# mlpc-ucsd/BDM

Measured on AMD Instinct MI355X. Metric: sampled shapes/sec (4096 pts, 1000 DDPM steps), higher is better.
Workload: dtype f32

## Files before the change

bdm_amd/csrc/sparse_conv_os.hip:

```cpp
#include <stdlib.h>

#include "../../include/bdm_hip.h"
#include "common.h"

using namespace bdm;

#include "sparse_h2_common.h"

#define OS_PAIRS 14

typedef __attribute__((ext_vector_type(4))) float f32x4a;
typedef float f32x4v_t __attribute__((ext_vector_type(4)));


#define TILE_REC 16
#define DILH_XCAP 1376

static void sconv_dil_geometry(int r, int half_tile, int *tile, int *xcap, int *tiles_max) {
  if (half_tile > 0) {
    *tile = half_tile;
    *xcap = DILH_XCAP;
  } else {
    *tile = r == 32 ? 512 : (r == 16 ? 256 : 128);
    *xcap = 3 * r * r;
  }
  *tiles_max = (r * r * r) / *tile + r;
}

__global__ __launch_bounds__(1024) void vox_dilate_kernel(int r, int n_dil_max, int tile, int xcap, int tiles_max, int half_form,
                                                          const int *__restrict__ cnt, int thr, int *__restrict__ dil_list,
                                                          int *__restrict__ dil_index, int *__restrict__ plane_start,
                                                          int *__restrict__ tile_start, int *__restrict__ class_count) {
  extern __shared__ unsigned bits[];
  const int bi = blockIdx.x, tid = threadIdx.x, T = blockDim.x, lane = tid & 63, wave = tid >> 6;
  const int r2 = r * r, r3 = r2 * r;
  unsigned *occ = bits;
  int *wtot = reinterpret_cast<int *>(bits + r2);
  int *ps_o = wtot + 32, *ps_d = ps_o + (r + 2);
  const int *c = cnt + (size_t)bi * r3;
  for (int v0 = wave * 64; v0 < r3; v0 += 8 * T) {
    int cv[8];
#pragma unroll
    for (int u = 0; u < 8; ++u) cv[u] = v0 + u * T < r3 ? c[v0 + u * T + lane] : thr;
#pragma unroll
    for (int u = 0; u < 8; ++u) {
      const int vu = v0 + u * T;
      if (vu < r3) {
        const unsigned long long m = __ballot(cv[u] > thr);
        const int rows = 64 / r;
        if (lane < rows) occ[vu / r + lane] = (unsigned)((m >> (lane * r)) & (r == 32 ? 0xffffffffull : ((1ull << r) - 1ull)));
      }
    }
  }
  __syncthreads();
  const unsigned full = r == 32 ? 0xffffffffu : ((1u << r) - 1u);
  unsigned d = 0u;
  int nocc_row = 0;
  if (tid < r2) {
    const int x = tid / r, y = tid % r;
    for (int dx = -1; dx <= 1; ++dx)
      for (int dy = -1; dy <= 1; ++dy) {
        const int gx = x + dx, gy = y + dy;
        if (gx < 0 || gx >= r || gy < 0 || gy >= r) continue;
        const unsigned m = occ[gx * r + gy];
        d |= m | (m << 1) | (m >> 1);
      }
    d &= full;
    nocc_row = __popc(occ[tid]);
  }
  int incl_d = __popc(d), incl_o = nocc_row;
  const int mine_d = incl_d, mine_o = incl_o;
#pragma unroll
  for (int o = 1; o < 64; o <<= 1) {
    const int td = __shfl_up(incl_d, o, 64), to = __shfl_up(incl_o, o, 64);
    if (lane >= o) { incl_d += td; incl_o += to; }
  }
  if (lane == 63) { wtot[wave] = incl_d; wtot[16 + wave] = incl_o; }
  __syncthreads();
  int off_d = 0, off_o = 0, tot_d = 0, tot_o = 0;
  for (int w = 0; w < (T >> 6); ++w) {
    if (w < wave) { off_d += wtot[w]; off_o += wtot[16 + w]; }
    tot_d += wtot[w]; tot_o += wtot[16 + w];
  }
  unsigned *drow = bits + r2 + 32 + 2 * (r + 2);
  int *drun = reinterpret_cast<int *>(drow + r2);
  int *rs = drun + r2;
  if (tid < r2) {
    const int run = off_d + incl_d - mine_d;
    if (tid % r == 0) { ps_o[tid / r] = off_o + incl_o - mine_o; ps_d[tid / r] = run; }
    drow[tid] = d;
    drun[tid] = run;
    rs[tid] = off_o + incl_o - mine_o;
  }
  if (tid == 0) rs[r2] = tot_o;
  __syncthreads();
  {
    int *dl = dil_list + (size_t)bi * n_dil_max;
    int *di = dil_index + (size_t)bi * r3;
    for (int v = tid; v < r3; v += T) {
      const int row = v / r, z = v - row * r;
      const unsigned m = drow[row];
      const bool in = (m >> z) & 1u;
      const int rank = drun[row] + __popc(m & ((1u << z) - 1u));
      const bool ok = in && rank < n_dil_max;
      di[v] = ok ? rank : -1;
      if (ok) dl[rank] = v;
    }
  }
  if (class_count != nullptr) {
    __shared__ int s_cls[27];
    if (tid < 27) s_cls[tid] = 0;
    __syncthreads();
    if (tid < r2) {
      const int x = tid / r, y = tid % r;
      const int cx = x == 0 ? 0 : (x == r - 1 ? 2 : 1), cy = y == 0 ? 0 : (y == r - 1 ? 2 : 1);
      const unsigned out = ~d & full;
      const int lo = out & 1u, hi = (out >> (r - 1)) & 1u, mid = __popc(out) - lo - hi;
      if (lo) atomicAdd(&s_cls[(cx * 3 + cy) * 3 + 0], lo);
      if (mid) atomicAdd(&s_cls[(cx * 3 + cy) * 3 + 1], mid);
      if (hi) atomicAdd(&s_cls[(cx * 3 + cy) * 3 + 2], hi);
    }
    __syncthreads();
    if (tid < 27) class_count[(size_t)bi * 27 + tid] = s_cls[tid];
  }
  if (tid == 0) { ps_o[r] = ps_o[r + 1] = tot_o; ps_d[r] = ps_d[r + 1] = tot_d; }
  __syncthreads();
  for (int x = tid; x < r + 2; x += T) plane_start[(size_t)bi * (r + 2) + x] = ps_o[x];
  if (half_form) {
    __threadfence();
    __syncthreads();
    const int *dl = dil_list + (size_t)bi * n_dil_max;
    const int nd = min(tot_d, n_dil_max), nt_flat = (nd + tile - 1) / tile;
    int pieces = 0, j = 0, jend = 0, x0 = 0, x1 = 0;
    if (tid < nt_flat) {
      j = tid * tile; jend = min(j + tile, nd);
      x0 = dl[j] / r2; x1 = dl[jend - 1] / r2;
      pieces = (x0 == x1 || rs[min(x1 + 2, r) * r] - rs[max(x0 - 1, 0) * r] <= xcap) ? 1 : x1 - x0 + 1;
    }
    int incl = pieces;
#pragma unroll
    for (int o = 1; o < 64; o <<= 1) {
      const int tq = __shfl_up(incl, o, 64);
      if (lane >= o) incl += tq;
    }
    if (lane == 63) wtot[wave] = incl;
    __syncthreads();
    int off = 0, nt = 0;
    for (int w = 0; w < (T >> 6); ++w) {
      if (w < wave) off += wtot[w];
      nt += wtot[w];
    }
    nt = min(nt, tiles_max);
    off += incl - pieces;
    for (int k = 0; k < pieces; ++k) {
      const int t = off + k;
      if (t >= tiles_max) break;
      int a = j, e_ = jend, xa = x0, xb = x1;
      if (pieces > 1) { xa = xb = x0 + k; a = max(j, ps_d[xa]); e_ = min(jend, ps_d[xa + 1]); if (e_ < a) e_ = a; }
      int lo[3] = {0, 0, 0}, nn[3] = {0, 0, 0};
      if (e_ > a) {
        if (xa == xb) {
          const int y0 = (dl[a] / r) % r, y1 = (dl[e_ - 1] / r) % r;
          for (int dx = 0; dx < 3; ++dx) {
            const int px = xa + dx - 1;
            if (px < 0 || px >= r) continue;
            lo[dx] = rs[px * r + max(y0 - 1, 0)];
            nn[dx] = rs[px * r + min(y1 + 1, r - 1) + 1] - lo[dx];
          }
        } else {
          lo[0] = rs[max(xa - 1, 0) * r];
          nn[0] = rs[min(xb + 2, r) * r] - lo[0];
        }
      }
      int *e = tile_start + ((size_t)bi * tiles_max + t) * TILE_REC;
      const int vf = t == 0 ? 0 : (a < nd ? dl[a] : r3), ve = (t + 1 < nt && e_ < nd) ? dl[e_] : r3;
      e[0] = a; e[1] = e_; e[2] = vf; e[3] = ve; e[4] = lo[0]; e[5] = nn[0]; e[6] = (xa << 8) | xb; e[7] = nt;
      e[8] = lo[1]; e[9] = nn[1]; e[10] = lo[2]; e[11] = nn[2]; e[12] = tile; e[13] = e[14] = e[15] = 0;
    }
    for (int t = nt + tid; t < tiles_max; t += T) {
      int *e = tile_start + ((size_t)bi * tiles_max + t) * TILE_REC;
      const bool first_empty = t == 0;
      e[0] = nd; e[1] = nd; e[2] = first_empty ? 0 : r3; e[3] = r3; e[4] = 0; e[5] = 0; e[6] = 0; e[7] = nt;
      for (int q = 8; q < TILE_REC; ++q) e[q] = q == 12 ? tile : 0;
    }
    return;
  }
  int *tinfo = reinterpret_cast<int *>(occ);
  __shared__ int s_tiles, s_cut;
  if (tid == 0) s_cut = 0;
  __syncthreads();
  {
    const int nd = min(tot_d, n_dil_max), nt_flat = (nd + tile - 1) / tile;
    if (tid < nt_flat && tid < tiles_max) {
      const int j = tid * tile, jend = min(j + tile, nd);
      int lo = 0, hi = r;
      while (hi - lo > 1) { const int mid = (lo + hi) >> 1; if (ps_d[mid] <= j) lo = mid; else hi = mid; }
      const int x0 = lo;
      lo = x0; hi = r;
      while (hi - lo > 1) { const int mid = (lo + hi) >> 1; if (ps_d[mid] <= jend - 1) lo = mid; else hi = mid; }
      const int x1 = lo;
      if (x1 > x0 && ps_o[min(x1 + 2, r)] - ps_o[max(x0 - 1, 0)] > xcap) s_cut = 1;
      tinfo[2 * tid] = j; tinfo[2 * tid + 1] = (x0 << 8) | x1;
    }
    if (tid == 0) { tinfo[2 * min(nt_flat, tiles_max)] = nd; s_tiles = min(nt_flat, tiles_max); }
  }
  __syncthreads();
  if (tid == 0 && s_cut) {
    const int nd = min(tot_d, n_dil_max);
    int t = 0, j = 0, x0 = 0;
    while (j < nd && t < tiles_max) {
      while (ps_d[x0 + 1] <= j) ++x0;
      int jend = min(j + tile, nd), x1 = x0;
      while (ps_d[x1 + 1] < jend) ++x1;
      while (x1 > x0 && ps_o[min(x1 + 2, r)] - ps_o[max(x0 - 1, 0)] > xcap) { jend = ps_d[x1]; --x1; }
      tinfo[2 * t] = j; tinfo[2 * t + 1] = (x0 << 8) | x1;
      ++t;
      j = jend;
    }
    tinfo[2 * t] = nd;
    s_tiles = t;
  }
  __threadfence();
  __syncthreads();
  const int nt = s_tiles, nd = min(tot_d, n_dil_max);
  for (int t = tid; t < tiles_max; t += T) {
    int *e = tile_start + ((size_t)bi * tiles_max + t) * TILE_REC;
    const int *dl = dil_list + (size_t)bi * n_dil_max;
    int j0 = nd, jn = nd, vf = r3, ve = r3, klo = 0, nr = 0;
    if (t < nt) {
      j0 = tinfo[2 * t]; jn = tinfo[2 * t + 2];
      const int x0 = tinfo[2 * t + 1] >> 8, x1 = tinfo[2 * t + 1] & 255;
      vf = t == 0 ? 0 : dl[j0];
      ve = t + 1 < nt ? dl[jn] : r3;
      klo = ps_o[max(x0 - 1, 0)];
      nr = min(ps_o[min(x1 + 2, r)] - klo, xcap);
    } else if (t == 0) { vf = 0; ve = r3; }
    e[0] = j0; e[1] = jn; e[2] = vf; e[3] = ve; e[4] = klo; e[5] = nr; e[6] = t < nt ? tinfo[2 * t + 1] : 0; e[7] = nt;
    for (int q = 8; q < TILE_REC; ++q) e[q] = 0;
  }
}

#ifdef BDM_EXPERIMENTAL
static bool half_tile_ok(int r, int tile) { return tile == 0 || ((r == 16 || r == 32) && (tile == 64 || tile == 128 || tile == 256)) || (r == 8 && (tile == 64 || tile == 128)); }
#else
static bool half_tile_ok(int, int tile) { return tile == 0; }
#endif

extern "C" int bdm_voxel_dilate_slices(int r, int tile) {
  int tl, xcap, tiles_max;
  sconv_dil_geometry(r, half_tile_ok(r, tile) ? tile : 0, &tl, &xcap, &tiles_max);
  return tiles_max;
}

static int voxel_dilate_launch(int b, int r, int n_dil_max, const int *src, int thr, int *dil_list, int *dil_index, int *plane_start,
                               int *tile_start, int *class_count, int half_tile, void *stream) {
  BDM_REQUIRE(b >= 0 && (r == 8 || r == 16 || r == 32) && n_dil_max >= 1 && src && dil_list && dil_index && plane_start && tile_start,
              "voxel_dilate: bad arguments (r in {8, 16, 32})");
  BDM_REQUIRE(half_tile_ok(r, half_tile), "voxel_dilate: tile %d unsupported (0 = full tiles; 64 / 128 / 256: EXPERIMENTAL=1 builds)", half_tile);
  if (b == 0) return BDM_OK;
  int tile, xcap, tiles_max;
  sconv_dil_geometry(r, half_tile, &tile, &xcap, &tiles_max);
  BDM_REQUIRE(cdiv(r * r * r, tile) <= 1024, "voxel_dilate: more flat tiles than threads");
  const size_t smem = sizeof(unsigned) * (4 * (size_t)r * r + 1 + 32 + 2 * (r + 2));
  hipLaunchKernelGGL(vox_dilate_kernel, dim3(b), dim3(1024), smem, (hipStream_t)stream, r, n_dil_max, tile, xcap, tiles_max,
                     half_tile > 0 ? 1 : 0, src, thr, dil_list, dil_index, plane_start, tile_start, class_count);
  return launch_status("voxel_dilate");
}

extern "C" int bdm_voxel_dilate(int b, int r, int n_dil_max, const int *cnt, int *dil_list, int *dil_index, int *plane_start,
                                int *tile_start, int tile, void *stream) {
  return voxel_dilate_launch(b, r, n_dil_max, cnt, 0, dil_list, dil_index, plane_start, tile_start, nullptr, tile, stream);
}

extern "C" int bdm_voxel_dilate_again(int b, int r, int n_dil_max, const int *dil_index_in, int *dil_list, int *dil_index,
                                      int *plane_start, int *tile_start, int *class_count, int tile, void *stream) {
  BDM_REQUIRE(class_count != nullptr, "voxel_dilate_again: class_count is NULL");
  return voxel_dilate_launch(b, r, n_dil_max, dil_index_in, -1, dil_list, dil_index, plane_start, tile_start, class_count, tile, stream);
}

#ifdef DIL_TIMING
__device__ long long *g_dil_ts = nullptr;
extern "C" int bdm_debug_dil_timestamps(long long *buf) { return hipMemcpyToSymbol(HIP_SYMBOL(g_dil_ts), &buf, sizeof(buf)) == hipSuccess ? 0 : 1; }
#define DIL_STAMP(i) do { if (g_dil_ts && tid == 0) { g_dil_ts[(size_t)item * 8 + (i)] = wall_clock64();                                  \
    if ((i) == 0) g_dil_ts[(size_t)item * 8 + 7] = (long long)__builtin_amdgcn_s_getreg(63492) | ((long long)__builtin_amdgcn_s_getreg(63508) << 32); } } while (0)
#else
#define DIL_STAMP(i)
#endif

template <int MT, int NT, int NW, int R, bool H2IN>
__global__ __launch_bounds__(NW * 64) void sconv_dil_kernel(
    int C8, int Cout, int n_max, int n_dil_max, int xcap, const float4 *__restrict__ xr, const float *__restrict__ amax,
    const float4 *__restrict__ xconst, float x_inv_scale,
    const int *__restrict__ occ_index, const int *__restrict__ dil_list, const int *__restrict__ dil_index,
    const int *__restrict__ tile_start, const float4 *__restrict__ wq,
    const float *__restrict__ inv_scale, const float *__restrict__ bias, float *__restrict__ y, int compact, int gn_cg,
    double *__restrict__ gn_partial, int gn_slices, int nb_shapes, int ncb, int tiles_max, int *__restrict__ work_counter) {
  extern __shared__ __align__(16) float4 smem4[];
  constexpr int BM = 16 * MT, TILE = NT * NW * 16;
  constexpr int R2 = R * R, R3 = R2 * R;
  constexpr int NT_ = NW * 64;
  constexpr int WV = OS_PAIRS * 2 * 2 * BM, WI = (WV + NT_ - 1) / NT_;
  constexpr int NQ = OS_PAIRS / 2;
  constexpr int PF = MT * NT >= 16 ? 1 : 2;
  constexpr int NBLK = NT * NW, NB = MT * 4 * 2;
  float4 *Ws = smem4;
  float4 *Xs = smem4 + WV;
  const int XS = xcap + 128;
  __shared__ int s_item;
  __shared__ float s_osc[64], s_obi[64];

  const int tid0 = threadIdx.x;
  const int G = gn_partial != nullptr ? Cout / gn_cg : 0, S = gn_slices;
  const int items = tiles_max * ncb * nb_shapes;
  for (;;) {
    int tid = tid0;
    asm volatile("" : "+v"(tid));
    const int lane = tid & 63, wave = tid >> 6, l16 = lane & 15, kg = lane >> 4;
    __syncthreads();
    if (tid == 0) s_item = atomicAdd(work_counter, 1);
    __syncthreads();
    const int item = s_item;
    if (item >= items) break;
    const int bi = item % nb_shapes, m0 = ((item / nb_shapes) % ncb) * BM, tile = item / (nb_shapes * ncb);
  const int4 *te = reinterpret_cast<const int4 *>(tile_start + ((size_t)bi * tiles_max + tile) * TILE_REC);
  const int4 ta = te[0], tb = te[1];
  const int j0 = ta.x, jn = ta.y, v_first = ta.z, v_end = ta.w, k_lo = tb.x;
  const int tiles_live = tb.w, tile_x0 = tb.z >> 8, tile_x1 = tb.z & 255;
  if (tile >= max(tiles_live, 1)) {
    if (gn_partial != nullptr) {
      const int ngt = BM / gn_cg;
      if (tid < ngt && m0 + tid * gn_cg < Cout) {
        double *dst = gn_partial + (((size_t)bi * G + m0 / gn_cg + tid) * S + tile) * 2;
        dst[0] = 0.0; dst[1] = 0.0;
      }
    }
    continue;
  }
  DIL_STAMP(0);
  const int *dl = dil_list + (size_t)bi * n_dil_max;
  const bool nothing = jn <= j0;
  const int nrows = nothing ? 0 : tb.y;

  const float sx = H2IN ? 1.0f / x_inv_scale : act_scale_from_max(amax[bi]);
  if (tid < BM) {
    const int m = min(m0 + tid, Cout - 1);
    s_osc[tid] = inv_scale[m] * (1.0f / sx);
    s_obi[tid] = bias ? bias[m] : 0.f;
  }
  const float4 *wbase = Ws + ((kg >> 1) * 4 + (kg & 1)) * BM + l16;
  f32x4a acc[MT][NT];
#pragma unroll
  for (int a = 0; a < MT; ++a)
#pragma unroll
    for (int q = 0; q < NT; ++q) acc[a][q] = f32x4a{0.f, 0.f, 0.f, 0.f};
  f32x4v_t cr = {0.f, 0.f, 0.f, 0.f};

  const float4 *xb = xr + (size_t)bi * C8 * n_max * 2;
  typedef f32x4v_t f32x4v;
  f32x4v xa[PF][2], wr[WI];
  auto load_chunk = [&](int c8) {
#pragma unroll
    for (int u = 0; u < PF; ++u) {
      const int row = min(tid + u * NT_, max(nrows - 1, 0));
      if (H2IN) {
        const f32x4v *src = reinterpret_cast<const f32x4v *>(xr + (((size_t)bi * C8 + c8) * 2) * n_max + k_lo + row);
        xa[u][0] = src[0];
        xa[u][1] = src[n_max];
      } else {
        const f32x4v *src = reinterpret_cast<const f32x4v *>(xb + ((size_t)c8 * n_max + k_lo + row) * 2);
        xa[u][0] = src[0];
        xa[u][1] = src[1];
      }
    }
    if (H2IN && tid < 128) cr = *reinterpret_cast<const f32x4v *>(xconst + ((size_t)bi * C8 + c8) * 2 + (tid >> 6));
#pragma unroll
    for (int i = 0; i < WI; ++i) {
      const int e = tid + i * NT_;
      const int m = e % BM, psh = e / BM;
      const bool ok = e < WV && m0 + m < Cout;
      wr[i] = *reinterpret_cast<const f32x4v *>(&wq[ok ? (unsigned)((c8 * (OS_PAIRS * 4) + psh) * Cout + m0 + m) : 0u]);
    }
  };
  auto put = [&](int row, const float4 &p, const float4 &q) {
    if (H2IN) {
      Xs[row] = p;
      Xs[XS + row] = q;
    } else {
      f16x8 hi, lo;
      split_record(p, q, sx, hi, lo);
      *reinterpret_cast<f16x8 *>(&Xs[row]) = hi;
      *reinterpret_cast<f16x8 *>(&Xs[XS + row]) = lo;
    }
  };
  auto store_chunk = [&](int c8) {
#pragma unroll
    for (int u = 0; u < PF; ++u)
      if (tid + u * NT_ < nrows) {
        const float4 p = make_float4(xa[u][0][0], xa[u][0][1], xa[u][0][2], xa[u][0][3]);
        const float4 q = make_float4(xa[u][1][0], xa[u][1][1], xa[u][1][2], xa[u][1][3]);
        put(tid + u * NT_, p, q);
      }
    for (int row0 = tid + PF * NT_; row0 < nrows; row0 += 2 * NT_) {
      const int row1 = row0 + NT_, rc1 = min(row1, nrows - 1);
      float4 a0, a1, b0, b1;
      if (H2IN) {
        const float4 *src = xr + (((size_t)bi * C8 + c8) * 2) * n_max + k_lo;
        a0 = src[row0]; a1 = src[n_max + row0]; b0 = src[rc1]; b1 = src[n_max + rc1];
      } else {
        const float4 *src = xb + ((size_t)c8 * n_max + k_lo) * 2;
        a0 = src[2 * row0]; a1 = src[2 * row0 + 1]; b0 = src[2 * rc1]; b1 = src[2 * rc1 + 1];
      }
      put(row0, a0, a1);
      if (row1 < nrows) put(row1, b0, b1);
    }
    if (H2IN && tid < 128) *reinterpret_cast<f32x4v *>(&Xs[(tid >> 6) * XS + xcap + 64 + (tid & 63)]) = cr;
#pragma unroll
    for (int i = 0; i < WI; ++i) {
      const int e = tid + i * NT_;
      if (e < WV) *reinterpret_cast<f32x4v *>(&Ws[e]) = wr[i];
    }
  };

  if (!nothing) load_chunk(0);

  int rec[NT][NQ];
  unsigned amask = 0u;
  {
    const int pl0 = max(tile_x0 - 1, 0), pl1 = min(tile_x1 + 1, R - 1), n_oi = (pl1 - pl0 + 1) * R2;
    const bool staged = !nothing && n_oi * (int)sizeof(int) <= 2 * XS * (int)sizeof(float4);
    int *s_oi = reinterpret_cast<int *>(Xs);
    const int *oi = occ_index + (size_t)bi * R3;
    int vq[NT];
#pragma unroll
    for (int q = 0; q < NT; ++q) {
      const int j = j0 + (q * NW + wave) * 16 + l16;
      vq[q] = j < jn ? dl[j] : -1;
    }
    if (staged) {
      const int4 *src = reinterpret_cast<const int4 *>(oi + pl0 * R2);
      for (int e = tid; e < n_oi / 4; e += NT_) reinterpret_cast<int4 *>(s_oi)[e] = src[e];
      __syncthreads();
    }
#pragma unroll
    for (int q = 0; q < NT; ++q) {
      const int v = vq[q];
      const int vx = v / R2, vy = (v / R) % R, vz = v % R;
#pragma unroll
      for (int Q = 0; Q < NQ; ++Q) {
        const int t = 4 * Q + kg;
        int k = -1;
        bool inside = false;
        if (v >= 0 && t < 27) {
          const int gx = vx + t / 9 - 1, gy = vy + (t / 3) % 3 - 1, gz = vz + t % 3 - 1;
          inside = gx >= 0 && gx < R && gy >= 0 && gy < R && gz >= 0 && gz < R;
          if (inside) k = staged ? s_oi[((gx - pl0) * R + gy) * R + gz] : oi[(gx * R + gy) * R + gz];
        }
        const bool here = k >= k_lo && k - k_lo < nrows;
        const bool live = here || (H2IN && inside);
        if (__ballot(live) != 0ull) amask |= 1u << (Q * NT + q);
        rec[q][Q] = here ? k - k_lo : ((H2IN && inside) ? xcap + 64 + lane : xcap + lane);
      }
    }
    amask = __builtin_amdgcn_readfirstlane(amask);
  }
  DIL_STAMP(1);
  if (!nothing) {
    for (int c8 = 0; c8 < C8; ++c8) {
      __syncthreads();
      if (c8 == 0) DIL_STAMP(2);
      if (c8 == 0 && tid < 128) Xs[(tid >> 6) * XS + xcap + (tid & 63)] = make_float4(0.f, 0.f, 0.f, 0.f);
      store_chunk(c8);
      __syncthreads();
      if (c8 == 0) DIL_STAMP(3);
      if (c8 == 1) DIL_STAMP(4);
      if (c8 + 1 < C8) load_chunk(c8 + 1);
#pragma unroll
      for (int Q = 0; Q < NQ; ++Q) {
        const unsigned qm = (amask >> (Q * NT)) & ((1u << NT) - 1u);
        if (qm == 0u) continue;
        f16x8 fa[MT][2];
#pragma unroll
        for (int s = 0; s < 2; ++s)
#pragma unroll
          for (int mt = 0; mt < MT; ++mt) {
            const float4 t = wbase[Q * 8 * BM + s * 2 * BM + mt * 16];
            fa[mt][s] = *reinterpret_cast<const f16x8 *>(&t);
          }
#pragma unroll
        for (int q = 0; q < NT; ++q) {
          f16x8 fb[2];
#pragma unroll
          for (int s = 0; s < 2; ++s) {
            const float4 t = Xs[s * XS + rec[q][Q]];
            fb[s] = *reinterpret_cast<const f16x8 *>(&t);
          }
#pragma unroll
          for (int term = 0; term < 3; ++term)
#pragma unroll
            for (int mt = 0; mt < MT; ++mt)
              acc[mt][q] = __builtin_amdgcn_mfma_f32_16x16x32_f16(fa[mt][term == 0 ? 1 : 0], fb[term == 1 ? 1 : 0], acc[mt][q], 0, 0, 0);
        }
      }
    }
  }

  DIL_STAMP(5);
  __syncthreads();
  float *red = reinterpret_cast<float *>(smem4);
  float *otile = red + (NBLK + 1) * NB;
#pragma unroll
  for (int mt = 0; mt < MT; ++mt)
#pragma unroll
    for (int q = 0; q < NT; ++q) {
      const int jl = (q * NW + wave) * 16 + l16;
      const bool live = j0 + jl < jn;
      float bs = 0.f, bq = 0.f;
      f32x4a o = f32x4a{0.f, 0.f, 0.f, 0.f};
#pragma unroll
      for (int i = 0; i < 4; ++i) {
        const int m = m0 + mt * 16 + 4 * kg + i;
        if (m < Cout && live) {
          const float v = acc[mt][q][i] * s_osc[mt * 16 + 4 * kg + i] + s_obi[mt * 16 + 4 * kg + i];
          o[i] = v;
          bs += v;
          bq = __builtin_fmaf(v, v, bq);
        }
      }
      if (live) {
        const int mb = m0 + mt * 16 + 4 * kg;
        if (compact) {
          float *dst = y + ((size_t)bi * n_dil_max + j0 + jl) * Cout + mb;
          if (mb + 3 < Cout && (Cout & 3) == 0) *reinterpret_cast<f32x4a *>(dst) = o;
          else
            for (int i = 0; i < 4 && mb + i < Cout; ++i) dst[i] = o[i];
        } else {
#pragma unroll
          for (int i = 0; i < 4; ++i) otile[(mt * 16 + 4 * kg + i) * TILE + jl] = o[i];
        }
      }
      if (gn_partial != nullptr) {
        bs = row16_sum(bs);
        bq = row16_sum(bq);
        if (l16 == 0) {
          const int nb = q * NW + wave;
          red[nb * NB + (mt * 4 + kg) * 2 + 0] = bs;
          red[nb * NB + (mt * 4 + kg) * 2 + 1] = bq;
        }
      }
    }
  if (gn_partial != nullptr || !compact) __syncthreads();
  if (!compact) {
    const int *di = dil_index + (size_t)bi * R3;
    float *yb = y + (size_t)bi * Cout * R3;
    for (int m = wave; m < BM; m += NW) {
      if (m0 + m >= Cout) break;
      const float bv = bias ? bias[m0 + m] : 0.f;
      float *row = yb + (size_t)(m0 + m) * R3;
      for (int v = v_first + lane; v < v_end; v += 64) {
        const int j = di[v];
        row[v] = j >= 0 ? otile[m * TILE + (j - j0)] : bv;
      }
    }
  }
  if (gn_partial != nullptr) {
    float *red2 = red + NBLK * NB;
    for (int e = tid; e < NB; e += NT_) {
      float a = 0.f;
#pragma unroll
      for (int j = 0; j < NBLK; ++j) a += red[j * NB + e];
      red2[e] = a;
    }
    __syncthreads();
    const int ngt = BM / gn_cg;
    if (tid < ngt && m0 + tid * gn_cg < Cout) {
      double a = 0.0, qq = 0.0;
      const int nb4 = gn_cg / 4;
      for (int j = 0; j < nb4; ++j) {
        a += (double)red2[(tid * nb4 + j) * 2 + 0];
        qq += (double)red2[(tid * nb4 + j) * 2 + 1];
      }
      const double nfill = H2IN ? 0.0 : (double)((v_end - v_first) - (jn - j0));
      for (int c = 0; c < gn_cg; ++c) {
        const double bv = bias ? (double)bias[m0 + tid * gn_cg + c] : 0.0;
        a += nfill * bv;
        qq += nfill * bv * bv;
      }
      double *dst = gn_partial + (((size_t)bi * G + m0 / gn_cg + tid) * S + tile) * 2;
      dst[0] = a;
      dst[1] = qq;
    }
  }
  DIL_STAMP(6);
  }
}


#ifdef BDM_EXPERIMENTAL
template <int MT, int NT, int R, bool H2IN>
__global__ __launch_bounds__(256, 2) void sconv_dilh_kernel(
    int C8, int Cout, int n_max, int n_dil_max, const float4 *__restrict__ xr, const float *__restrict__ amax,
    const float4 *__restrict__ xconst, float x_inv_scale,
    const int *__restrict__ occ_index, const int *__restrict__ dil_list, const int *__restrict__ dil_index,
    const int *__restrict__ tile_start, const float4 *__restrict__ wq,
    const float *__restrict__ inv_scale, const float *__restrict__ bias, float *__restrict__ y, int compact, int gn_cg,
    double *__restrict__ gn_partial, int gn_slices, int nb_shapes, int ncb, int tiles_max, int *__restrict__ work_counter) {
  extern __shared__ __align__(16) float4 smem4[];
  constexpr int NW = 4, NT_ = NW * 64;
  constexpr int BM = 16 * MT, TILE = NT * NW * 16;
  constexpr int R2 = R * R, R3 = R2 * R;
  constexpr int NQ = OS_PAIRS / 2;
  constexpr int PF = 3;
  constexpr int NBLK = NT * NW, NB = MT * 4 * 2;
  constexpr int XCAP = DILH_XCAP, XS = XCAP + 128;
  float4 *Xs = smem4;
  __shared__ int s_item;
  __shared__ float s_osc[64], s_obi[64];

  const int tid0 = threadIdx.x;
  const int G = gn_partial != nullptr ? Cout / gn_cg : 0, S = gn_slices;
  const int items = tiles_max * ncb * nb_shapes;
  for (;;) {
    int tid = tid0;
    asm volatile("" : "+v"(tid));
    const int lane = tid & 63, wave = tid >> 6, l16 = lane & 15, kg = lane >> 4;
    __syncthreads();
    if (tid == 0) s_item = atomicAdd(work_counter, 1);
    __syncthreads();
    const int item = s_item;
    if (item >= items) break;
    const int bi = item % nb_shapes, m0 = ((item / nb_shapes) % ncb) * BM, tile = item / (nb_shapes * ncb);
    const int4 *te = reinterpret_cast<const int4 *>(tile_start + ((size_t)bi * tiles_max + tile) * TILE_REC);
    const int4 ta = te[0], tb = te[1], tc = te[2];
    const int j0 = ta.x, jn = ta.y, v_first = ta.z, v_end = ta.w;
    const int tiles_live = tb.w, tile_x0 = tb.z >> 8, tile_x1 = tb.z & 255;
    if (tile >= max(tiles_live, 1)) {
      if (gn_partial != nullptr) {
        const int ngt = BM / gn_cg;
        if (tid < ngt && m0 + tid * gn_cg < Cout) {
          double *dst = gn_partial + (((size_t)bi * G + m0 / gn_cg + tid) * S + tile) * 2;
          dst[0] = 0.0; dst[1] = 0.0;
        }
      }
      continue;
    }
    DIL_STAMP(0);
    const int *dl = dil_list + (size_t)bi * n_dil_max;
    const bool nothing = jn <= j0;
    const int lo0 = tb.x, n0 = nothing ? 0 : tb.y, lo1 = tc.x, n1 = nothing ? 0 : tc.y, lo2 = tc.z, n2 = nothing ? 0 : tc.w;
    const int n01 = n0 + n1, nrows = min(n01 + n2, XCAP);
    auto grow = [&](int i) { return i < n0 ? lo0 + i : (i < n01 ? lo1 + (i - n0) : lo2 + (i - n01)); };

    const float sx = H2IN ? 1.0f / x_inv_scale : act_scale_from_max(amax[bi]);
    if (tid < BM) {
      const int m = min(m0 + tid, Cout - 1);
      s_osc[tid] = inv_scale[m] * (1.0f / sx);
      s_obi[tid] = bias ? bias[m] : 0.f;
    }
    const __amdgpu_buffer_rsrc_t wrsrc = __builtin_amdgcn_make_buffer_rsrc(const_cast<float4 *>(wq), 0, C8 * (OS_PAIRS * 4) * Cout * 16, 0x00020000);
    const int wlane = (((kg >> 1) * 4 + (kg & 1)) * Cout + m0 + l16) * 16;
    f32x4a acc[MT][NT];
#pragma unroll
    for (int a = 0; a < MT; ++a)
#pragma unroll
      for (int q = 0; q < NT; ++q) acc[a][q] = f32x4a{0.f, 0.f, 0.f, 0.f};
    typedef f32x4v_t f32x4v;
    f32x4v cr = {0.f, 0.f, 0.f, 0.f};
    f32x4v xa[PF][2];
    const float4 *xb = xr + (size_t)bi * C8 * n_max * 2;

    auto load_x = [&](int c8) {
#pragma unroll
      for (int u = 0; u < PF; ++u) {
        const int g = grow(min(tid + u * NT_, max(nrows - 1, 0)));
        if (H2IN) {
          const f32x4v *src = reinterpret_cast<const f32x4v *>(xr + (((size_t)bi * C8 + c8) * 2) * n_max + g);
          xa[u][0] = src[0];
          xa[u][1] = src[n_max];
        } else {
          const f32x4v *src = reinterpret_cast<const f32x4v *>(xb + ((size_t)c8 * n_max + g) * 2);
          xa[u][0] = src[0];
          xa[u][1] = src[1];
        }
      }
      if (H2IN && tid < 128) cr = *reinterpret_cast<const f32x4v *>(xconst + ((size_t)bi * C8 + c8) * 2 + (tid >> 6));
    };
    auto put = [&](int row, const float4 &p, const float4 &q) {
      if (H2IN) {
        Xs[row] = p;
        Xs[XS + row] = q;
      } else {
        f16x8 hi, lo;
        split_record(p, q, sx, hi, lo);
        *reinterpret_cast<f16x8 *>(&Xs[row]) = hi;
        *reinterpret_cast<f16x8 *>(&Xs[XS + row]) = lo;
      }
    };
    auto store_x = [&](int c8) {
      const int rows_w = nrows;
#pragma unroll
      for (int u = 0; u < PF; ++u)
        if (tid + u * NT_ < rows_w) {
          const float4 p = make_float4(xa[u][0][0], xa[u][0][1], xa[u][0][2], xa[u][0][3]);
          const float4 q = make_float4(xa[u][1][0], xa[u][1][1], xa[u][1][2], xa[u][1][3]);
          put(tid + u * NT_, p, q);
        }
      for (int row0 = tid + PF * NT_; row0 < rows_w; row0 += 2 * NT_) {
        const int row1 = row0 + NT_, rc1 = min(row1, rows_w - 1);
        const int g0 = grow(row0), g1 = grow(rc1);
        float4 a0, a1, b0, b1;
        if (H2IN) {
          const float4 *src = xr + (((size_t)bi * C8 + c8) * 2) * n_max;
          a0 = src[g0]; a1 = src[n_max + g0]; b0 = src[g1]; b1 = src[n_max + g1];
        } else {
          const float4 *src = xb + ((size_t)c8 * n_max) * 2;
          a0 = src[2 * g0]; a1 = src[2 * g0 + 1]; b0 = src[2 * g1]; b1 = src[2 * g1 + 1];
        }
        put(row0, a0, a1);
        if (row1 < rows_w) put(row1, b0, b1);
      }
      if (H2IN && tid < 128) *reinterpret_cast<f32x4v *>(&Xs[(tid >> 6) * XS + XCAP + 64 + (tid & 63)]) = cr;
    };

    if (!nothing) load_x(0);

    int rec[NT][NQ];
    unsigned amask = 0u;
    {
      const int pl0 = max(tile_x0 - 1, 0), pl1 = min(tile_x1 + 1, R - 1), n_oi = (pl1 - pl0 + 1) * R2;
      const bool staged = !nothing && n_oi * (int)sizeof(int) <= 2 * XS * (int)sizeof(float4);
      int *s_oi = reinterpret_cast<int *>(Xs);
      const int *oi = occ_index + (size_t)bi * R3;
      int vq[NT];
#pragma unroll
      for (int q = 0; q < NT; ++q) {
        const int j = j0 + (q * NW + wave) * 16 + l16;
        vq[q] = j < jn ? dl[j] : -1;
      }
      if (staged) {
        const int4 *src = reinterpret_cast<const int4 *>(oi + pl0 * R2);
        for (int e = tid; e < n_oi / 4; e += NT_) reinterpret_cast<int4 *>(s_oi)[e] = src[e];
        __syncthreads();
      }
#pragma unroll
      for (int q = 0; q < NT; ++q) {
        const int v = vq[q];
        const int vx = v / R2, vy = (v / R) % R, vz = v % R;
#pragma unroll
        for (int Q = 0; Q < NQ; ++Q) {
          const int t = 4 * Q + kg;
          int k = -1;
          bool inside = false;
          if (v >= 0 && t < 27) {
            const int gx = vx + t / 9 - 1, gy = vy + (t / 3) % 3 - 1, gz = vz + t % 3 - 1;
            inside = gx >= 0 && gx < R && gy >= 0 && gy < R && gz >= 0 && gz < R;
            if (inside) k = staged ? s_oi[((gx - pl0) * R + gy) * R + gz] : oi[(gx * R + gy) * R + gz];
          }
          int row = -1;
          if (k >= 0) {
            if ((unsigned)(k - lo0) < (unsigned)n0) row = k - lo0;
            else if ((unsigned)(k - lo1) < (unsigned)n1) row = n0 + (k - lo1);
            else if ((unsigned)(k - lo2) < (unsigned)n2) row = n01 + (k - lo2);
          }
          const bool here = row >= 0 && row < XCAP;
          const bool cst = H2IN && inside && !here;
          if (__ballot(here || cst) != 0ull) amask |= 1u << (Q * NT + q);
          rec[q][Q] = here ? row : (cst ? XCAP + 64 + lane : XCAP + lane);
        }
      }
      amask = __builtin_amdgcn_readfirstlane(amask);
    }
    DIL_STAMP(1);

    if (!nothing) {
      f32x4v fa[MT][2], fn[MT][2];
      auto load_a = [&](f32x4v (&dst)[MT][2], int c8, int Q) {
        const int so = ((c8 * NQ + Q) * 8) * Cout * 16;
#pragma unroll
        for (int s = 0; s < 2; ++s)
#pragma unroll
          for (int mt = 0; mt < MT; ++mt)
            dst[mt][s] = __builtin_bit_cast(f32x4v, __builtin_amdgcn_raw_buffer_load_b128(wrsrc, wlane + mt * 256, so + s * 2 * Cout * 16, 0));
      };
      const unsigned live_q = [&] {
        unsigned m = 0u;
#pragma unroll
        for (int Q = 0; Q < NQ; ++Q)
          if ((amask >> (Q * NT)) & ((1u << NT) - 1u)) m |= 1u << Q;
        return m;
      }();
      int q_first = 0;
      while (q_first < NQ && !((live_q >> q_first) & 1u)) ++q_first;
      if (q_first < NQ) load_a(fa, 0, q_first);
      for (int c8 = 0; c8 < C8; ++c8) {
        __syncthreads();
        if (c8 == 0) DIL_STAMP(2);
        if (c8 == 0 && tid < 128) Xs[(tid >> 6) * XS + XCAP + (tid & 63)] = make_float4(0.f, 0.f, 0.f, 0.f);
        store_x(c8);
        lds_barrier();
        if (c8 == 0) DIL_STAMP(3);
        if (c8 == 1) DIL_STAMP(4);
        if (c8 + 1 < C8) load_x(c8 + 1);
#pragma unroll
        for (int Q = 0; Q < NQ; ++Q) {
          if (!((live_q >> Q) & 1u)) continue;
          {
            int nq = Q + 1;
            while (nq < NQ && !((live_q >> nq) & 1u)) ++nq;
            if (nq < NQ) load_a(fn, c8, nq);
            else if (c8 + 1 < C8) load_a(fn, c8 + 1, q_first);
          }
#pragma unroll
          for (int q = 0; q < NT; ++q) {
            f16x8 fb[2];
#pragma unroll
            for (int s = 0; s < 2; ++s) {
              const float4 t = Xs[s * XS + rec[q][Q]];
              fb[s] = *reinterpret_cast<const f16x8 *>(&t);
            }
#pragma unroll
            for (int term = 0; term < 3; ++term)
#pragma unroll
              for (int mt = 0; mt < MT; ++mt)
                acc[mt][q] = __builtin_amdgcn_mfma_f32_16x16x32_f16(__builtin_bit_cast(f16x8, fa[mt][term == 0 ? 1 : 0]), fb[term == 1 ? 1 : 0],
                                                                    acc[mt][q], 0, 0, 0);
          }
#pragma unroll
          for (int s = 0; s < 2; ++s)
#pragma unroll
            for (int mt = 0; mt < MT; ++mt) fa[mt][s] = fn[mt][s];
        }
      }
    }

    DIL_STAMP(5);
    __syncthreads();
    float *red = reinterpret_cast<float *>(smem4);
    float *otile = red + (NBLK + 1) * NB;
#pragma unroll
    for (int mt = 0; mt < MT; ++mt)
#pragma unroll
      for (int q = 0; q < NT; ++q) {
        const int jl = (q * NW + wave) * 16 + l16;
        const bool live = j0 + jl < jn;
        float bs = 0.f, bq = 0.f;
        f32x4a o = f32x4a{0.f, 0.f, 0.f, 0.f};
#pragma unroll
        for (int i = 0; i < 4; ++i) {
          const int m = m0 + mt * 16 + 4 * kg + i;
          if (m < Cout && live) {
            const float v = acc[mt][q][i] * s_osc[mt * 16 + 4 * kg + i] + s_obi[mt * 16 + 4 * kg + i];
            o[i] = v;
            bs += v;
            bq = __builtin_fmaf(v, v, bq);
          }
        }
        if (live) {
          const int mb = m0 + mt * 16 + 4 * kg;
          if (compact) {
            float *dst = y + ((size_t)bi * n_dil_max + j0 + jl) * Cout + mb;
            if (mb + 3 < Cout && (Cout & 3) == 0) *reinterpret_cast<f32x4a *>(dst) = o;
            else
              for (int i = 0; i < 4 && mb + i < Cout; ++i) dst[i] = o[i];
          } else {
#pragma unroll
            for (int i = 0; i < 4; ++i) otile[(mt * 16 + 4 * kg + i) * TILE + jl] = o[i];
          }
        }
        if (gn_partial != nullptr) {
          bs = row16_sum(bs);
          bq = row16_sum(bq);
          if (l16 == 0) {
            const int nb = q * NW + wave;
            red[nb * NB + (mt * 4 + kg) * 2 + 0] = bs;
            red[nb * NB + (mt * 4 + kg) * 2 + 1] = bq;
          }
        }
      }
    if (gn_partial != nullptr || !compact) __syncthreads();
    if (!compact) {
      const int *di = dil_index + (size_t)bi * R3;
      float *yb = y + (size_t)bi * Cout * R3;
      for (int m = wave; m < BM; m += NW) {
        if (m0 + m >= Cout) break;
        const float bv = bias ? bias[m0 + m] : 0.f;
        float *row = yb + (size_t)(m0 + m) * R3;
        for (int v = v_first + lane; v < v_end; v += 64) {
          const int j = di[v];
          row[v] = (j >= j0 && j < jn) ? otile[m * TILE + (j - j0)] : bv;
        }
      }
    }
    if (gn_partial != nullptr) {
      float *red2 = red + NBLK * NB;
      for (int e = tid; e < NB; e += NT_) {
        float a = 0.f;
#pragma unroll
        for (int j = 0; j < NBLK; ++j) a += red[j * NB + e];
        red2[e] = a;
      }
      __syncthreads();
      const int ngt = BM / gn_cg;
      if (tid < ngt && m0 + tid * gn_cg < Cout) {
        double a = 0.0, qq = 0.0;
        const int nb4 = gn_cg / 4;
        for (int j = 0; j < nb4; ++j) {
          a += (double)red2[(tid * nb4 + j) * 2 + 0];
          qq += (double)red2[(tid * nb4 + j) * 2 + 1];
        }
        const double nfill = H2IN ? 0.0 : (double)((v_end - v_first) - (jn - j0));
        for (int c = 0; c < gn_cg; ++c) {
          const double bv = bias ? (double)bias[m0 + tid * gn_cg + c] : 0.0;
          a += nfill * bv;
          qq += nfill * bv * bv;
        }
        double *dst = gn_partial + (((size_t)bi * G + m0 / gn_cg + tid) * S + tile) * 2;
        dst[0] = a;
        dst[1] = qq;
      }
    }
    DIL_STAMP(6);
  }
}

#endif

static int sconv_dil_launch(bool h2in, int b, int cin, int cout, int r, int n_max, int n_dil_max, const void *xr, const float *amax,
                            const void *xconst, float x_inv_scale, const int *in_index, const int *dil_list, const int *dil_index,
                            const int *tile_start, const void *packed_w, const float *inv_scale, const float *bias, float *y,
                            int compact, int gn_cg, double *gn_partial, int *slices_out, int half_tile, int *work_counter,
                            void *stream) {
  BDM_REQUIRE(b >= 0 && cin >= 1 && cout >= 1 && n_max >= 1 && n_dil_max >= 1 && xr && (h2in ? xconst != nullptr : amax != nullptr) &&
                  in_index && dil_list && dil_index && tile_start && inv_scale && y && work_counter,
              "sparse_conv_dil: bad arguments");
  if (r != 8 && r != 16 && r != 32) {
    set_error("sparse_conv_dil: resolution %d unsupported (8, 16, 32)", r);
    return BDM_ERR_UNSUPPORTED;
  }
  BDM_REQUIRE(half_tile_ok(r, half_tile), "sparse_conv_dil: tile %d unsupported (0 = full tiles; 64 / 128 / 256: EXPERIMENTAL=1 builds)", half_tile);
  if (b == 0) return BDM_OK;
  const int c8 = (cin + 7) / 8;
  const int mi = cout > 32 ? 2 : 1;
  int tile, xcap, tiles;
  sconv_dil_geometry(r, half_tile, &tile, &xcap, &tiles);
  const int bm = 32 * mi, nblk = tile / 16, nb = (bm / 16) * 8, ncb = cdiv(cout, bm);
  size_t smem = half_tile ? 16 * (2 * ((size_t)xcap + 128))
                          : 16 * ((size_t)OS_PAIRS * 4 * bm + 2 * ((size_t)xcap + 128));
  const size_t smem_out = sizeof(float) * ((size_t)(nblk + 1) * nb + (compact ? 0 : (size_t)bm * tile));
  if (smem_out > smem) smem = smem_out;
  BDM_REQUIRE(!half_tile || smem + 1024 <= 81920, "sparse_conv_dil: the half-tile form needs two workgroups per CU (%zu bytes of LDS)", smem);
  static int cus[16] = {0};
  int dev = 0;
  (void)hipGetDevice(&dev);
  if (dev < 0 || dev >= 16 || cus[dev] == 0) {
    hipDeviceProp_t prop;
    const int n = hipGetDeviceProperties(&prop, dev) == hipSuccess ? prop.multiProcessorCount : 256;
    if (dev >= 0 && dev < 16) cus[dev] = n > 0 ? n : 256;
  }
  const int ncu = ((dev >= 0 && dev < 16) ? cus[dev] : 256) * (half_tile ? 2 : 1);
  const long long items = (long long)tiles * ncb * b;
  dim3 grid((unsigned)(items < ncu ? items : ncu));
  hipStream_t s = (hipStream_t)stream;
  const int slices = h2in ? tiles + 27 : tiles;
  if (gn_partial != nullptr) {
    BDM_REQUIRE(gn_cg >= 4 && (gn_cg & (gn_cg - 1)) == 0 && bm % gn_cg == 0 && cout % gn_cg == 0,
                "sparse_conv_dil: GroupNorm statistics need a power-of-two channels-per-group dividing %d (got cg=%d)", bm, gn_cg);
    if (slices_out) *slices_out = slices;
  }
#define DIL_LAUNCH_(MT, NT, NW, R, H)                                                                                      \
  do {                                                                                                                     \
    BDM_ALLOW_LDS((sconv_dil_kernel<MT, NT, NW, R, H>), smem);                                                             \
    hipLaunchKernelGGL((sconv_dil_kernel<MT, NT, NW, R, H>), grid, dim3(NW * 64), smem, s, c8, cout, n_max, n_dil_max,     \
                       xcap, (const float4 *)xr, amax, (const float4 *)xconst, x_inv_scale, in_index, dil_list, dil_index, \
                       tile_start, (const float4 *)packed_w, inv_scale, bias, y, compact, gn_cg, gn_partial, slices, b,    \
                       ncb, tiles, work_counter);                                                                          \
  } while (0)
#define DIL_LAUNCH(MT, NT, NW, R) do { if (h2in) DIL_LAUNCH_(MT, NT, NW, R, true); else DIL_LAUNCH_(MT, NT, NW, R, false); } while (0)
#define DILH_LAUNCH_(MT, NT, R, H)                                                                                         \
  do {                                                                                                                     \
    BDM_ALLOW_LDS((sconv_dilh_kernel<MT, NT, R, H>), smem);                                                                \
    hipLaunchKernelGGL((sconv_dilh_kernel<MT, NT, R, H>), grid, dim3(256), smem, s, c8, cout, n_max, n_dil_max,            \
                       (const float4 *)xr, amax, (const float4 *)xconst, x_inv_scale, in_index, dil_list, dil_index,       \
                       tile_start, (const float4 *)packed_w, inv_scale, bias, y, compact, gn_cg, gn_partial, slices, b,    \
                       ncb, tiles, work_counter);                                                                          \
  } while (0)
#define DILH_LAUNCH(MT, NT, R) do { if (h2in) DILH_LAUNCH_(MT, NT, R, true); else DILH_LAUNCH_(MT, NT, R, false); } while (0)
#define DILH_PICK(NT, R) do { if (mi == 2) DILH_LAUNCH(4, NT, R); else DILH_LAUNCH(2, NT, R); } while (0)
#ifdef BDM_EXPERIMENTAL
  if (half_tile) {
    const int nt = half_tile / 64;
    if (r == 32) { if (nt == 4) DILH_PICK(4, 32); else if (nt == 2) DILH_PICK(2, 32); else DILH_PICK(1, 32); }
    else if (r == 16) { if (nt == 4) DILH_PICK(4, 16); else if (nt == 2) DILH_PICK(2, 16); else DILH_PICK(1, 16); }
    else { if (nt == 2) DILH_PICK(2, 8); else DILH_PICK(1, 8); }
    return launch_status("sparse_conv_dil (half tiles)");
  }
#endif
  if (r == 32) { if (mi == 2) DIL_LAUNCH(4, 4, 8, 32); else DIL_LAUNCH(2, 4, 8, 32); }
  else if (r == 16) { if (mi == 2) DIL_LAUNCH(4, 2, 8, 16); else DIL_LAUNCH(2, 2, 8, 16); }
  else { if (mi == 2) DIL_LAUNCH(4, 1, 8, 8); else DIL_LAUNCH(2, 1, 8, 8); }
#undef DIL_LAUNCH
#undef DIL_LAUNCH_
#undef DILH_PICK
#undef DILH_LAUNCH
#undef DILH_LAUNCH_
  return launch_status("sparse_conv_dil");
}

extern "C" int bdm_sparse_conv_dil(int b, int cin, int cout, int r, int n_max, int n_dil_max, const void *xr, const float *amax,
                                   const int *occ_index, const int *dil_list, const int *dil_index, const int *tile_start,
                                   const void *packed_w, const float *inv_scale, const float *bias, float *y,
                                   int compact, int tile, int *work_counter, void *stream) {
  return sconv_dil_launch(false, b, cin, cout, r, n_max, n_dil_max, xr, amax, nullptr, 0.f, occ_index, dil_list, dil_index, tile_start,
                          packed_w, inv_scale, bias, y, compact, 0, nullptr, nullptr, tile, work_counter, stream);
}

extern "C" int bdm_sparse_conv_dil_gn(int b, int cin, int cout, int r, int n_max, int n_dil_max, const void *xr, const float *amax,
                                      const int *occ_index, const int *dil_list, const int *dil_index, const int *tile_start,
                                      const void *packed_w, const float *inv_scale, const float *bias,
                                      float *y, int compact, int groups, void *gn_partial, int *slices_out, int tile,
                                      int *work_counter, void *stream) {
  BDM_REQUIRE(groups >= 1 && cout % groups == 0 && gn_partial != nullptr && slices_out != nullptr, "sparse_conv_dil_gn: bad arguments");
  return sconv_dil_launch(false, b, cin, cout, r, n_max, n_dil_max, xr, amax, nullptr, 0.f, occ_index, dil_list, dil_index, tile_start,
                          packed_w, inv_scale, bias, y, compact, cout / groups, (double *)gn_partial, slices_out, tile, work_counter, stream);
}

extern "C" int bdm_sparse_conv_dil_h2_gn(int b, int cin, int cout, int r, int n_rows_max, int n_dil_max, const void *rows_h2,
                                         const void *xconst, float x_inv_scale, const int *in_index, const int *dil_list,
                                         const int *dil_index, const int *tile_start, const void *packed_w, const float *inv_scale,
                                         const float *bias, float *y, int groups, void *gn_partial, int *slices_out, int tile,
                                         int *work_counter, void *stream) {
  BDM_REQUIRE(groups >= 1 && cout % groups == 0 && gn_partial != nullptr && slices_out != nullptr && x_inv_scale > 0.f,
              "sparse_conv_dil_h2_gn: bad arguments");
  return sconv_dil_launch(true, b, cin, cout, r, n_rows_max, n_dil_max, rows_h2, nullptr, xconst, x_inv_scale, in_index, dil_list,
                          dil_index, tile_start, packed_w, inv_scale, bias, y, 1, cout / groups, (double *)gn_partial, slices_out, tile,
                          work_counter, stream);
}
```

Baseline: 3.105.

## Batch occupancy lookups, unroll index staging, vectorize epilogue scale/bias loads

The occupancy-index staging loop now issues four independent 16-byte loads per thread before storing them. The neighbor lookup is split into two passes, all gathers first and then classification and ballot, so memory latency can overlap. The epilogue loads per-channel scale and bias once as float4 vectors, swaps the loop order to q-outer, and simplifies the vector store condition. The GroupNorm fill term now reads bias from shared s_obi instead of global memory. That is only correct if s_obi equals the raw bias for those channels.

```diff
diff --git a/bdm_amd/csrc/sparse_conv_os.hip b/bdm_amd/csrc/sparse_conv_os.hip
--- a/bdm_amd/csrc/sparse_conv_os.hip
+++ b/bdm_amd/csrc/sparse_conv_os.hip
@@ -307,7 +307,7 @@
   float4 *Xs = smem4 + WV;
   const int XS = xcap + 128;
   __shared__ int s_item;
-  __shared__ float s_osc[64], s_obi[64];
+  __shared__ __align__(16) float s_osc[64], s_obi[64];
 
   const int tid0 = threadIdx.x;
   const int G = gn_partial != nullptr ? Cout / gn_cg : 0, S = gn_slices;
@@ -438,29 +438,47 @@
     }
     if (staged) {
       const int4 *src = reinterpret_cast<const int4 *>(oi + pl0 * R2);
-      for (int e = tid; e < n_oi / 4; e += NT_) reinterpret_cast<int4 *>(s_oi)[e] = src[e];
+      int4 *dst = reinterpret_cast<int4 *>(s_oi);
+      const int n4 = n_oi / 4;
+      for (int e = tid; e < n4; e += 4 * NT_) {
+        int4 p[4];
+#pragma unroll
+        for (int u = 0; u < 4; ++u) p[u] = src[min(e + u * NT_, n4 - 1)];
+#pragma unroll
+        for (int u = 0; u < 4; ++u)
+          if (e + u * NT_ < n4) dst[e + u * NT_] = p[u];
+      }
       __syncthreads();
     }
-#pragma unroll
-    for (int q = 0; q < NT; ++q) {
-      const int v = vq[q];
-      const int vx = v / R2, vy = (v / R) % R, vz = v % R;
-#pragma unroll
-      for (int Q = 0; Q < NQ; ++Q) {
-        const int t = 4 * Q + kg;
-        int k = -1;
-        bool inside = false;
-        if (v >= 0 && t < 27) {
-          const int gx = vx + t / 9 - 1, gy = vy + (t / 3) % 3 - 1, gz = vz + t % 3 - 1;
-          inside = gx >= 0 && gx < R && gy >= 0 && gy < R && gz >= 0 && gz < R;
-          if (inside) k = staged ? s_oi[((gx - pl0) * R + gy) * R + gz] : oi[(gx * R + gy) * R + gz];
-        }
-        const bool here = k >= k_lo && k - k_lo < nrows;
-        const bool live = here || (H2IN && inside);
-        if (__ballot(live) != 0ull) amask |= 1u << (Q * NT + q);
-        rec[q][Q] = here ? k - k_lo : ((H2IN && inside) ? xcap + 64 + lane : xcap + lane);
-      }
-    }
+    auto inside_at = [&](int q, int Q, int &gx, int &gy, int &gz) {
+      const int v = vq[q], t = 4 * Q + kg;
+      gx = v / R2 + t / 9 - 1; gy = (v / R) % R + (t / 3) % 3 - 1; gz = v % R + t % 3 - 1;
+      return v >= 0 && t < 27 && gx >= 0 && gx < R && gy >= 0 && gy < R && gz >= 0 && gz < R;
+    };
+    auto lookup = [&](auto &&cell) {
+#pragma unroll
+      for (int q = 0; q < NT; ++q)
+#pragma unroll
+        for (int Q = 0; Q < NQ; ++Q) {
+          int gx, gy, gz;
+          const bool inside = inside_at(q, Q, gx, gy, gz);
+          rec[q][Q] = cell(inside ? gx : pl0, inside ? gy : 0, inside ? gz : 0);
+        }
+#pragma unroll
+      for (int q = 0; q < NT; ++q)
+#pragma unroll
+        for (int Q = 0; Q < NQ; ++Q) {
+          int gx, gy, gz;
+          const bool inside = inside_at(q, Q, gx, gy, gz);
+          const int k = inside ? rec[q][Q] : -1;
+          const bool here = k >= k_lo && k - k_lo < nrows;
+          const bool live = here || (H2IN && inside);
+          amask |= (__ballot(live) != 0ull ? 1u : 0u) << (Q * NT + q);
+          rec[q][Q] = here ? k - k_lo : ((H2IN && inside) ? xcap + 64 + lane : xcap + lane);
+        }
+    };
+    if (staged) lookup([&](int gx, int gy, int gz) { return s_oi[((gx - pl0) * R + gy) * R + gz]; });
+    else lookup([&](int gx, int gy, int gz) { return oi[(gx * R + gy) * R + gz]; });
     amask = __builtin_amdgcn_readfirstlane(amask);
   }
   DIL_STAMP(1);
@@ -508,30 +526,37 @@
   __syncthreads();
   float *red = reinterpret_cast<float *>(smem4);
   float *otile = red + (NBLK + 1) * NB;
-#pragma unroll
-  for (int mt = 0; mt < MT; ++mt)
-#pragma unroll
-    for (int q = 0; q < NT; ++q) {
-      const int jl = (q * NW + wave) * 16 + l16;
-      const bool live = j0 + jl < jn;
+  f32x4a osc[MT], obi[MT];
+#pragma unroll
+  for (int mt = 0; mt < MT; ++mt) {
+    osc[mt] = *reinterpret_cast<const f32x4a *>(&s_osc[mt * 16 + 4 * kg]);
+    obi[mt] = *reinterpret_cast<const f32x4a *>(&s_obi[mt * 16 + 4 * kg]);
+  }
+  const bool vec4 = (Cout & 3) == 0;
+#pragma unroll
+  for (int q = 0; q < NT; ++q) {
+    const int jl = (q * NW + wave) * 16 + l16;
+    const bool live = j0 + jl < jn;
+    float *yrow = y + ((size_t)bi * n_dil_max + j0 + jl) * Cout + m0 + 4 * kg;
+#pragma unroll
+    for (int mt = 0; mt < MT; ++mt) {
       float bs = 0.f, bq = 0.f;
-      f32x4a o = f32x4a{0.f, 0.f, 0.f, 0.f};
+      f32x4a o;
 #pragma unroll
       for (int i = 0; i < 4; ++i) {
-        const int m = m0 + mt * 16 + 4 * kg + i;
-        if (m < Cout && live) {
-          const float v = acc[mt][q][i] * s_osc[mt * 16 + 4 * kg + i] + s_obi[mt * 16 + 4 * kg + i];
-          o[i] = v;
-          bs += v;
-          bq = __builtin_fmaf(v, v, bq);
-        }
+        const bool ok = m0 + mt * 16 + 4 * kg + i < Cout && live;
+        const float v = acc[mt][q][i] * osc[mt][i] + obi[mt][i];
+        o[i] = ok ? v : 0.f;
+        bs += o[i];
+        bq = __builtin_fmaf(o[i], o[i], bq);
       }
       if (live) {
         const int mb = m0 + mt * 16 + 4 * kg;
         if (compact) {
-          float *dst = y + ((size_t)bi * n_dil_max + j0 + jl) * Cout + mb;
-          if (mb + 3 < Cout && (Cout & 3) == 0) *reinterpret_cast<f32x4a *>(dst) = o;
-          else
+          float *dst = yrow + mt * 16;
+          if (vec4) {
+            if (mb < Cout) *reinterpret_cast<f32x4a *>(dst) = o;
+          } else
             for (int i = 0; i < 4 && mb + i < Cout; ++i) dst[i] = o[i];
         } else {
 #pragma unroll
@@ -548,6 +573,7 @@
         }
       }
     }
+  }
   if (gn_partial != nullptr || !compact) __syncthreads();
   if (!compact) {
     const int *di = dil_index + (size_t)bi * R3;
@@ -581,7 +607,7 @@
       }
       const double nfill = H2IN ? 0.0 : (double)((v_end - v_first) - (jn - j0));
       for (int c = 0; c < gn_cg; ++c) {
-        const double bv = bias ? (double)bias[m0 + tid * gn_cg + c] : 0.0;
+        const double bv = (double)s_obi[tid * gn_cg + c];
         a += nfill * bv;
         qq += nfill * bv * bv;
       }
```

Result: no change. 3.132, median of 6 (+0.9%).
